# adobe/3D-FM-GAN

Measured on AMD Instinct MI355X. Metric: (photo,render) pairs/sec, higher is better.
Workload: dtype f32; 1 GPU; pairs1024: cfg4 shard: E_Tsr+E_W+E_W_Plus(18 styles) on 256^2 -> co-mod -> Generator(1024) forward, fp32, B=8/GPU; pairs_per_gpu=8, global_pairs=8, image_size=1024, parallelism=replicas x1 (batch-sharded, no collective), launch=eager, ranks=1, full=False

## Files before the change

3d-fm-gan_amd/csrc/modconv_fwd.hip:

```cpp
#include <type_traits>
#include "common.h"
#include <cstdio>
#include <cstdlib>

namespace {

typedef unsigned u32x2 __attribute__((ext_vector_type(2)));

template <int SIZE, typename RSRC>
__device__ __forceinline__ void dma_to_lds(RSRC rsrc, float* lds, unsigned voff, unsigned soff) {
#if defined(__HIP_DEVICE_COMPILE__)
  typedef __attribute__((address_space(3))) void* lds_void_ptr;
  __builtin_amdgcn_raw_ptr_buffer_load_lds(rsrc, (lds_void_ptr)lds, SIZE, voff, soff, 0, 0);
#endif
}

__device__ __forceinline__ const float* uniform_ptr(const float* q) {
  const unsigned long long v = (unsigned long long)q;
  const unsigned lo = __builtin_amdgcn_readfirstlane((unsigned)v), hi = __builtin_amdgcn_readfirstlane((unsigned)(v >> 32));
  return (const float*)(((unsigned long long)hi << 32) | lo);
}
__device__ __forceinline__ unsigned uniform_u32(unsigned v) { return __builtin_amdgcn_readfirstlane(v); }

struct MCParams {
  const float* in; const float* wt; const float* style; const float* demod; float* out;
  int batch, cin, cout, h, w, oh, ow;
  long long out_plane_stride; int out_row_stride;
  struct Seg {
    int m_off, n_off, gh, gw;
    int th, nb, tw_log2;
    int tiles_x, tiles_y, tiles_b;
    unsigned block_end;
    int wide;
  } seg[3];
  int nseg, o_tiles;
  int ksplit, cin_per_split;
  float* ws;
  const float* noise; const float* noise_weight; const float* bias;
  int noise_batch, fuse_act; float alpha, act_scale;
  const float* rgb_wmod;
  const float* rgb_bias; const float* rgb_skip; float* rgb_out;
  int rgb_c;
  int lds_buf_floats, lds_patch_floats;
  int lds_style_floats;
  int debug;
  unsigned long long* dbg_clock;
  int exp_flags;
};

#ifdef FMGAN_EXPERIMENTS
#define MC_DEBUG(p) ((p).debug)
#define MC_CLOCK(p) ((p).dbg_clock)
#define MC_FLAGS(p) ((p).exp_flags)
#else
#define MC_DEBUG(p) 0
#define MC_CLOCK(p) false
#define MC_FLAGS(p) 0
#endif

constexpr int MC_KC = 8;

__device__ __forceinline__ float mc_epilogue(float v, const MCParams& p, float nw, int b, int o, int pix) {
  if (p.demod) v *= p.demod[(long long)b * p.cout + o];
  if (p.fuse_act) {
    const float n = p.noise ? p.noise[(long long)(p.noise_batch == 1 ? 0 : b) * p.oh * p.ow + pix] : 0.f;
    const float bv = p.bias ? p.bias[o] : 0.f;
    v = __fadd_rn(__fadd_rn(v, __fmul_rn(nw, n)), bv);
    v = (v > 0.f ? v : v * p.alpha) * p.act_scale;
  }
  return v;
}

template <int MODE_, int RM_, int RNP_, int WM_, int WN_, int MINB_, int KC_, int PIPE_>
struct TileShape {
  static constexpr int MODE = MODE_, RM = RM_, RNP = RNP_, WM = WM_, WN = WN_, MINB = MINB_, KC = KC_, PIPE = PIPE_;
  static constexpr int BM = 32 * RM * WM, BN = 32 * RNP * WN;
};
struct Plain128x128Reg         : TileShape<   0,  2,   2,  2,  2,    2, MC_KC,    0> {};
struct Plain128x128DmaKc4      : TileShape<   0,  2,   2,  2,  2,    3,     4,    1> {};
struct Plain128x256DmaKc4      : TileShape<   0,  4,   2,  1,  4,    2,     4,    1> {};
struct Plain64x128Reg          : TileShape<   0,  2,   1,  1,  4,    3, MC_KC,    0> {};
struct Plain64x128Dma          : TileShape<   0,  2,   1,  1,  4,    3,     8,    1> {};
struct Plain64x256DmaKc4       : TileShape<   0,  2,   2,  1,  4,    3,     4,    1> {};
struct Plain32x128Reg          : TileShape<   0,  1,   1,  1,  4,    4, MC_KC,    0> {};
struct Plain32x128Dma          : TileShape<   0,  1,   1,  1,  4,    4,     8,    1> {};
struct Plain32x256DmaKc4R128   : TileShape<   0,  1,   2,  1,  4,    4,     4,    1> {};
struct Stride2x128x128Reg      : TileShape<   2,  2,   2,  2,  2,    2, MC_KC,    0> {};
struct Stride2x64x128Reg       : TileShape<   2,  2,   1,  1,  4,    2, MC_KC,    0> {};
struct Stride2x32x128Reg       : TileShape<   2,  1,   1,  1,  4,    2, MC_KC,    0> {};
struct Transposed64x128Reg     : TileShape<   1,  2,   1,  1,  4,    2, MC_KC,    0> {};
struct Transposed64x128Dma     : TileShape<   1,  2,   1,  1,  4,    2,     8,    1> {};
struct Transposed32x128Reg     : TileShape<   1,  1,   1,  1,  4,    3, MC_KC,    0> {};
struct Transposed32x128DmaR128 : TileShape<   1,  1,   1,  1,  4,    4,     8,    1> {};
#ifdef FMGAN_EXPERIMENTS
struct Plain32x256Dma          : TileShape<   0,  1,   2,  1,  4,    3,     8,    1> {};
struct Plain32x256DmaKc4R96    : TileShape<   0,  1,   2,  1,  4,    5,     4,    1> {};
struct Transposed32x256Dma     : TileShape<   1,  1,   2,  1,  4,    2,     8,    1> {};
struct Transposed32x128DmaR170 : TileShape<   1,  1,   1,  1,  4,    3,     8,    1> {};
#endif

template <class Tile, bool RGB>
__global__ __launch_bounds__(256, Tile::MINB) void modconv_mfma_f32(const MCParams p) {
  constexpr int MODE = Tile::MODE, RM = Tile::RM, RNP = Tile::RNP, WM = Tile::WM, WN = Tile::WN, KC = Tile::KC, PIPE = Tile::PIPE;
  static_assert(!RGB || MODE == 0, "the RGB epilogue belongs to the plain conv");
  static_assert(PIPE == 1 || KC == MC_KC, "the register pipeline is built for 8-channel chunks");
  constexpr int BM = Tile::BM;
  constexpr int NPH = MODE == 1 ? 4 : 1;
  static_assert(WM * WN == 4, "4 waves per block");
  extern __shared__ float smem[];
  float* Ws = smem;
  float* Xs = smem + KC * 9 * BM;

  const int tid = threadIdx.x, lane = tid & 63, wave = __builtin_amdgcn_readfirstlane(tid >> 6);
  const int wm = wave / WN, wn = wave % WN;
  const int l31 = lane & 31, khalf = lane >> 5;
  unsigned long long clk0 = 0, rt0 = 0;
  if (MC_CLOCK(p)) { clk0 = __builtin_readcyclecounter(); rt0 = wall_clock64(); }
  if (MC_FLAGS(p) & 1) __builtin_amdgcn_s_setprio(3);

  unsigned lb = xcd_remap(blockIdx.x, gridDim.x);
  int si = 0;
  while (si + 1 < p.nseg && lb >= p.seg[si].block_end) ++si;
  if (si > 0) lb -= p.seg[si - 1].block_end;
  const unsigned tapmask = (MODE == 1 && p.nseg == 3) ? (si == 0 ? 0x1C0u : (si == 1 ? 0x124u : 0x1FFu)) : 0x1FFu;
  const int seg_th = p.seg[si].th, seg_nb = p.seg[si].nb, tw_log2 = p.seg[si].tw_log2;
  const int seg_m_end = p.seg[si].m_off + p.seg[si].gh, seg_n_end = p.seg[si].n_off + p.seg[si].gw;
  constexpr int SP = MODE == 2 ? 2 : 1;
  constexpr int ORG = MODE == 2 ? 0 : 1;
  const bool wide = PIPE == 1 && SP == 1 && p.seg[si].wide != 0;
  const int XORG = wide ? 4 : ORG;
  const int TW = 1 << tw_log2, PWP = wide ? TW + 8 : SP * (TW - 1) + 3;
  const int o_tile = lb % p.o_tiles;
  unsigned pt = lb / p.o_tiles;
  const int tx_i = pt % p.seg[si].tiles_x; pt /= p.seg[si].tiles_x;
  const int ty_i = pt % p.seg[si].tiles_y;
  const int tb_i = pt / p.seg[si].tiles_y;
  const int ks = blockIdx.y;
  const int o0 = o_tile * BM, b0 = tb_i * seg_nb;
  const int x0 = p.seg[si].n_off + tx_i * TW, y0 = p.seg[si].m_off + ty_i * seg_th;
  const int PH = SP * (seg_th - 1) + 3;
  const int plane = PH * PWP;
  const int samp = KC * plane;

  int pbase[RNP], pos_b[RNP], pos_y[RNP], pos_x[RNP];
#pragma unroll
  for (int g = 0; g < RNP; ++g) {
    const int pos = (wn * RNP + g) * 32 + l31;
    const int tx = pos & (TW - 1), r = pos >> tw_log2;
    const int ty = r % seg_th, nbi = r / seg_th;
    pbase[g] = min(nbi, seg_nb - 1) * samp + SP * ty * PWP + SP * tx + (XORG - ORG);
    pos_b[g] = nbi < seg_nb ? b0 + nbi : p.batch; pos_y[g] = y0 + ty; pos_x[g] = x0 + tx;
  }

  f32x16 acc[RM][RNP][NPH];
#pragma unroll
  for (int a = 0; a < RM; ++a)
#pragma unroll
    for (int b = 0; b < RNP; ++b)
#pragma unroll
      for (int c = 0; c < NPH; ++c)
#pragma unroll
        for (int r = 0; r < 16; ++r) acc[a][b][c][r] = 0.f;

  const bool wvec = (p.cout & 3) == 0;
  const int i_begin = ks * p.cin_per_split;
  const int i_end = min(p.cin, i_begin + p.cin_per_split);
  const int hw = p.h * p.w;

  constexpr int BNP = 32 * RNP * WN;
  constexpr int NU = ((SP * (BNP / 32 - 1) + 3) * (SP * 31 + 3) + 255) / 256;
  constexpr int NWV = (KC * 9 * (BM / 4) + 255) / 256;
  const int spatial = seg_nb * plane;
  const float* in_b0 = uniform_ptr(p.in + (long long)b0 * p.cin * hw);
  const float* style_b0 = uniform_ptr(p.style + (long long)b0 * p.cin);
  const bool epi_lds = PIPE == 1 && seg_nb == 1 && p.ksplit == 1;
  float* Es = smem + 2 * p.lds_buf_floats;
  float epi_v = 0.f;
  if constexpr (PIPE == 1) {
    if (epi_lds && tid < 2 * BM) {
      const bool isd = tid >= BM;
      const int oc = min(o0 + (isd ? tid - BM : tid), p.cout - 1);
      epi_v = isd ? 1.f : 0.f;
      if (isd) { if (p.demod) epi_v = p.demod[(long long)min(b0, p.batch - 1) * p.cout + oc]; }
      else if (MODE == 0 && p.fuse_act && p.bias) epi_v = p.bias[oc];
    }
  }
  int gofs[NU], lofs[NU], sofs[NU]; bool inb[NU];
#pragma unroll
  for (int u = 0; u < NU; ++u) {
    const int q = tid + 256 * u;
    const int c = q % PWP;
    int t = q / PWP;
    const int r = t % PH, nbi = t / PH;
    const int b = b0 + nbi, y = SP * y0 + r - ORG, x = SP * x0 + c - ORG;
    inb[u] = q < spatial && b < p.batch && y >= 0 && y < p.h && x >= 0 && x < p.w;
    gofs[u] = inb[u] ? (nbi * p.cin * p.h + y) * p.w + x : 0;
    sofs[u] = nbi * p.cin;
    lofs[u] = q < spatial ? nbi * samp + r * PWP + c : -1;
  }
  float xv[NU][KC];
  f32x4 wv[NWV];
  constexpr long long PARK = 0xFFFFFFF0LL;
  const bool fastw = wvec && o0 + BM <= p.cout && (long long)p.cin * 9 * p.cout * 4 < PARK;
  const bool fastx = (long long)min(seg_nb, p.batch - b0) * p.cin * hw * 4 < PARK;
  const unsigned w_bytes = uniform_u32((unsigned)((long long)p.cin * 9 * p.cout * 4));
  const unsigned x_bytes = uniform_u32((unsigned)((long long)min(seg_nb, p.batch - b0) * p.cin * hw * 4));
  const auto rsrc_w = __builtin_amdgcn_make_buffer_rsrc(const_cast<float*>(p.wt), 0, w_bytes, 0x00020000);
  const auto rsrc_x = __builtin_amdgcn_make_buffer_rsrc(const_cast<float*>(in_b0), 0, x_bytes, 0x00020000);
  unsigned wofs[NWV], xofs[NU];
#pragma unroll
  for (int j = 0; j < NWV; ++j) {
    const int idx = tid + 256 * j;
    const int row = idx / (BM / 4), c4 = idx % (BM / 4);
    wofs[j] = idx < KC * 9 * (BM / 4) ? (unsigned)((row * p.cout + o0 + c4 * 4) * 4) : 0xFFFFFFF0u;
  }
#pragma unroll
  for (int u = 0; u < NU; ++u) xofs[u] = inb[u] ? (unsigned)gofs[u] * 4u : 0xFFFFFFF0u;
  auto issue = [&](int i0) {
    if (fastw && i0 + KC <= i_end) {
      const unsigned soff = (unsigned)(i0 * 9 * p.cout * 4);
#pragma unroll
      for (int j = 0; j < NWV; ++j) {
        const auto t = __builtin_amdgcn_raw_buffer_load_b128(rsrc_w, wofs[j], soff, 0);
        wv[j] = __builtin_bit_cast(f32x4, t);
      }
    } else {
#pragma unroll
      for (int j = 0; j < NWV; ++j) {
        const int idx = tid + 256 * j;
        const int row = idx / (BM / 4), c4 = idx % (BM / 4);
        const int i = i0 + row / 9, o = o0 + c4 * 4;
        f32x4 v = {0.f, 0.f, 0.f, 0.f};
        if (idx < KC * 9 * (BM / 4) && i < i_end) {
          const float* src = p.wt + ((long long)i * 9 + row % 9) * p.cout + o;
          if (wvec && o + 3 < p.cout) {
            v = *reinterpret_cast<const f32x4*>(src);
          } else {
            if (o + 0 < p.cout) v.x = src[0];
            if (o + 1 < p.cout) v.y = src[1];
            if (o + 2 < p.cout) v.z = src[2];
            if (o + 3 < p.cout) v.w = src[3];
          }
        }
        wv[j] = v;
      }
    }
    if (fastx && i0 + KC <= i_end) {
#pragma unroll
      for (int kc = 0; kc < KC; ++kc) {
        const unsigned soff = (unsigned)((i0 + kc) * hw * 4);
#pragma unroll
        for (int u = 0; u < NU; ++u)
          xv[u][kc] = __builtin_bit_cast(float, __builtin_amdgcn_raw_buffer_load_b32(rsrc_x, xofs[u], soff, 0));
      }
    } else {
#pragma unroll
      for (int u = 0; u < NU; ++u)
#pragma unroll
        for (int kc = 0; kc < KC; ++kc) {
          const int i = i0 + kc;
          xv[u][kc] = (inb[u] && i < i_end) ? in_b0[gofs[u] + i * hw] : 0.f;
        }
    }
  };
  auto commit = [&](int i0) {
#pragma unroll
    for (int j = 0; j < NWV; ++j) {
      const int idx = tid + 256 * j;
      if (idx < KC * 9 * (BM / 4)) *reinterpret_cast<f32x4*>(Ws + idx * 4) = wv[j];
    }
#pragma unroll
    for (int u = 0; u < NU; ++u)
      if (lofs[u] >= 0) {
        float sv[KC];
#pragma unroll
        for (int kc = 0; kc < KC; ++kc) sv[kc] = (inb[u] && i0 + kc < i_end) ? style_b0[sofs[u] + i0 + kc] : 0.f;
#pragma unroll
        for (int kc = 0; kc < KC; ++kc) Xs[lofs[u] + kc * plane] = xv[u][kc] * sv[kc];
      }
    for (int q = tid + 256 * NU; q < spatial; q += 256) {
      const int c = q % PWP;
      int t = q / PWP;
      const int r = t % PH, nbi = t / PH;
      const int b = b0 + nbi, y = SP * y0 + r - ORG, x = SP * x0 + c - ORG;
      const bool ok = b < p.batch && y >= 0 && y < p.h && x >= 0 && x < p.w;
      for (int kc = 0; kc < KC; ++kc) {
        const int i = i0 + kc;
        float v = 0.f;
        if (ok && i < i_end) {
          const long long ch = (long long)b * p.cin + i;
          v = p.in[(ch * p.h + y) * p.w + x] * p.style[ch];
        }
        Xs[nbi * samp + kc * plane + r * PWP + c] = v;
      }
    }
  };

  constexpr int NTA = MODE == 1 ? 9 : 3;
  constexpr int NTB = MODE == 1 ? 4 : 3;
  constexpr int NSTAGE = (KC / 2) * (MODE == 1 ? 1 : 3);
  struct Ops { float a[NTA][RM]; float b[NTB][RNP]; float s[RNP]; };
  const float* Wc = Ws;
  const float* Xc = Xs;
  const float* Sc = nullptr;
  int sbase[RNP];
#pragma unroll
  for (int g = 0; g < RNP; ++g) sbase[g] = (pbase[g] / samp) * KC;
  auto fetch = [&](Ops& o, int st) {
    const int kk = MODE == 1 ? st : st / 3, ky = MODE == 1 ? 0 : st % 3;
    const int kc = 2 * kk + khalf;
    const float* wrow = Wc + (kc * 9 + ky * 3) * BM + wm * 32 * RM + l31;
    const float* xrow = Xc + kc * plane;
#pragma unroll
    for (int t = 0; t < NTA; ++t)
#pragma unroll
      for (int m = 0; m < RM; ++m) o.a[t][m] = wrow[t * BM + m * 32];
    if constexpr (PIPE == 1) {
      if (MODE == 1 || ky == 0) {
#pragma unroll
        for (int g = 0; g < RNP; ++g) o.s[g] = Sc[sbase[g] + kc];
      }
    }
#pragma unroll
    for (int j = 0; j < NTB; ++j) {
      const int ro = MODE == 1 ? 1 - (j >> 1) : ky;
      const int co = MODE == 1 ? 1 - (j & 1) : j;
#pragma unroll
      for (int g = 0; g < RNP; ++g) o.b[j][g] = xrow[pbase[g] + ro * PWP + co];
    }
  };
  auto modulate = [&](Ops& o) {
    if constexpr (PIPE == 1) {
#pragma unroll
      for (int j = 0; j < NTB; ++j)
#pragma unroll
        for (int g = 0; g < RNP; ++g) o.b[j][g] *= o.s[g];
    }
  };
  auto mma = [&](const Ops& o, auto all_taps) {
// ... 35 lines not shown
        }
      }
      __builtin_amdgcn_sched_barrier(0);
      modulate(o0);
      __builtin_amdgcn_s_setprio(1);
      mma(o0, all_taps);
      __builtin_amdgcn_s_setprio(0);
      __builtin_amdgcn_sched_barrier(0);
      hook(st + 1);
      if (st + 2 < NSTAGE) {
        fetch(o0, st + 2);
        if constexpr (PIPE == 1 && MODE != 1) {
          if ((st + 2) % 3 != 0) {
#pragma unroll
            for (int g = 0; g < RNP; ++g) o0.s[g] = o1.s[g];
          }
        }
      }
      __builtin_amdgcn_sched_barrier(0);
      modulate(o1);
      __builtin_amdgcn_s_setprio(1);
      mma(o1, all_taps);
      __builtin_amdgcn_s_setprio(0);
      __builtin_amdgcn_sched_barrier(0);
    }
  };

  unsigned long long clk1 = 0, clk2 = 0, clkw = 0, clke = 0, clkl = 0;
  if (MC_CLOCK(p)) clk1 = __builtin_readcyclecounter();
  if (MC_FLAGS(p) & 1) __builtin_amdgcn_s_setprio(0);
  if constexpr (PIPE == 0) {
    if (i_begin < i_end) issue(i_begin);
    for (int i0 = i_begin; i0 < i_end; i0 += KC) {
      const bool live = !(MC_DEBUG(p) & 1) || i0 == i_begin;
      if (!(MC_DEBUG(p) & 2)) __syncthreads();
      if (live) commit(i0);
      if (!(MC_DEBUG(p) & 2)) __syncthreads();
      __builtin_amdgcn_sched_barrier(0);
      if (live && i0 + KC < i_end) issue(i0 + KC);
      contract([](int) {}, std::false_type{});
    }
  } else {
    constexpr unsigned PARKED = 0xFFFFFFF0u;
    constexpr int WSZ = (KC * 9 * BM + 255) / 256 * 256;
    constexpr int WPIECES = WSZ / 256;
    constexpr int NWP = (WPIECES + 3) / 4;
    constexpr int NUP = ((KC * (SP * (BNP / 32 - 1) + 3) * (SP * 31 + 3) + 63) / 64 + 3) / 4;
    const int xs_total = seg_nb * samp;
    const int x_piece_floats = wide ? 256 : 64;
    const int x_pieces = (xs_total + x_piece_floats - 1) / x_piece_floats;
    const int s_pieces = (seg_nb * KC + 63) >> 6;
    const int bstride = p.lds_buf_floats;
    const bool fastc = fastw && fastx;
    const unsigned s_bytes = (unsigned)(min(seg_nb, p.batch - b0) * p.cin * 4);
    const auto rsrc_s = __builtin_amdgcn_make_buffer_rsrc(const_cast<float*>(style_b0), 0, s_bytes, 0x00020000);
    auto x_voff = [&](int e) -> unsigned {
      if (e >= xs_total) return PARKED;
      const int nbi = e / samp, rem = e - nbi * samp;
      const int kc = rem / plane, q = rem - kc * plane;
      const int r = q / PWP, c = q - r * PWP;
      const int b = b0 + nbi, y = SP * y0 + r - ORG, x = SP * x0 + c - XORG;
      const bool ok = b < p.batch && y >= 0 && y < p.h && x >= 0 && x < p.w;
      return ok ? (unsigned)(((nbi * p.cin + kc) * p.h + y) * p.w + x) * 4u : PARKED;
    };
    auto x_voff16 = [&](int g16) -> unsigned { return x_voff(4 * g16); };
    auto s_voff = [&](int e) -> unsigned {
      const int nbi = e / KC, kc = e - nbi * KC;
      return (nbi < seg_nb && b0 + nbi < p.batch) ? (unsigned)(nbi * p.cin + kc) * 4u : PARKED;
    };
    unsigned wvo[NWP], xvo[NUP];
#pragma unroll
    for (int j = 0; j < NWP; ++j) {
      const int idx = (4 * j + wave) * 64 + lane;
      const int row = idx / (BM / 4), c4 = idx % (BM / 4);
      wvo[j] = idx < KC * 9 * (BM / 4) ? (unsigned)((row * p.cout + o0 + c4 * 4) * 4) : PARKED;
    }
#pragma unroll
    for (int u = 0; u < NUP; ++u)
      xvo[u] = 4 * u + wave < x_pieces ? (wide ? x_voff16((4 * u + wave) * 64 + lane) : x_voff((4 * u + wave) * 64 + lane)) : PARKED;
    const unsigned svo = s_voff(wave * 64 + lane);

    constexpr int NPC = NWP + NUP + 1;
    constexpr int PER_STAGE = (NPC + NSTAGE - 1) / NSTAGE;
    auto dma_piece = [&](int k, int i0, int buf) {
      float* Wb = smem + buf * bstride;
      float* Xb = Wb + WSZ;
      const unsigned soff_x = (unsigned)(i0 * hw * 4);
      if (k < NWP) {
        if (4 * k + wave < WPIECES)
          dma_to_lds<16>(rsrc_w, Wb + (4 * k + wave) * 256, wvo[k < NWP ? k : 0], (unsigned)(i0 * 9 * p.cout * 4));
      } else if (k < NWP + NUP) {
        const int u = k - NWP;
        if (4 * u + wave < x_pieces) {
          if (wide) dma_to_lds<16>(rsrc_x, Xb + (4 * u + wave) * 256, xvo[(u >= 0 && u < NUP) ? u : 0], soff_x);
          else dma_to_lds<4>(rsrc_x, Xb + (4 * u + wave) * 64, xvo[(u >= 0 && u < NUP) ? u : 0], soff_x);
        }
      } else {
        float* Sb = Xb + p.lds_patch_floats;
        for (int pc = 4 * NUP + wave; pc < x_pieces; pc += 4) {
          if (wide) dma_to_lds<16>(rsrc_x, Xb + pc * 256, x_voff16(pc * 64 + lane), soff_x);
          else dma_to_lds<4>(rsrc_x, Xb + pc * 64, x_voff(pc * 64 + lane), soff_x);
        }
        if (wave < s_pieces)
          dma_to_lds<4>(rsrc_s, Sb + wave * 64, svo, (unsigned)(i0 * 4));
        for (int pc = 4 + wave; pc < s_pieces; pc += 4)
          dma_to_lds<4>(rsrc_s, Sb + pc * 64, s_voff(pc * 64 + lane), (unsigned)(i0 * 4));
      }
    };
    auto dma_ok = [&](int i0) { return fastc && i0 + KC <= i_end; };

    auto stage = [&](int i0, int buf) {
      float* Wb = smem + buf * bstride;
      float* Xb = Wb + WSZ;
      float* Sb = Xb + p.lds_patch_floats;
      if (dma_ok(i0)) {
#pragma unroll
        for (int k = 0; k < NPC; ++k) dma_piece(k, i0, buf);
      } else {
        for (int idx = tid; idx < KC * 9 * (BM / 4); idx += 256) {
          const int row = idx / (BM / 4), c4 = idx % (BM / 4);
          const int i = i0 + row / 9, o = o0 + c4 * 4;
          f32x4 v = {0.f, 0.f, 0.f, 0.f};
          if (i < i_end) {
            const float* src = p.wt + ((long long)i * 9 + row % 9) * p.cout + o;
            if (o + 0 < p.cout) v.x = src[0];
            if (o + 1 < p.cout) v.y = src[1];
            if (o + 2 < p.cout) v.z = src[2];
            if (o + 3 < p.cout) v.w = src[3];
          }
          *reinterpret_cast<f32x4*>(Wb + idx * 4) = v;
        }
        for (int e = tid; e < x_pieces * x_piece_floats; e += 256) {
          float v = 0.f;
          if (e < xs_total) {
            const int nbi = e / samp, rem = e - nbi * samp;
            const int kc = rem / plane, q = rem - kc * plane;
            const int r = q / PWP, c = q - r * PWP;
            const int b = b0 + nbi, y = SP * y0 + r - ORG, x = SP * x0 + c - XORG, i = i0 + kc;
            if (b < p.batch && y >= 0 && y < p.h && x >= 0 && x < p.w && i < i_end)
              v = p.in[(((long long)b * p.cin + i) * p.h + y) * p.w + x];
          }
          Xb[e] = v;
        }
        for (int e = tid; e < seg_nb * KC; e += 256) {
          const int nbi = e / KC, kc = e - nbi * KC;
          Sb[e] = (b0 + nbi < p.batch && i0 + kc < i_end) ? p.style[(long long)(b0 + nbi) * p.cin + i0 + kc] : 0.f;
        }
      }
    };

    const bool lean = fastc && MC_DEBUG(p) == 0 && i_begin < i_end && ((i_end - i_begin) % KC) == 0 && x_pieces <= 4 * NUP &&
                      s_pieces <= 4 && tapmask == 0x1FFu;
    const bool style_once = lean && seg_nb == 1 && p.lds_style_floats > 0;
    float* Ss = Es + 2 * BM;
    if (lean) {
      auto piece = [&](int k, int i0, int bufi) {
        float* Wb = smem + bufi * bstride;
        float* Xb = Wb + WSZ;
        if (k < NWP) {
          if (WPIECES % 4 == 0 || 4 * k + wave < WPIECES)
            dma_to_lds<16>(rsrc_w, Wb + (4 * k + wave) * 256, wvo[k < NWP ? k : 0], (unsigned)(i0 * 9 * p.cout * 4));
        } else if (k < NWP + NUP) {
          const int u = k - NWP;
          if (4 * u + wave < x_pieces) {
            if (wide) dma_to_lds<16>(rsrc_x, Xb + (4 * u + wave) * 256, xvo[(u >= 0 && u < NUP) ? u : 0], (unsigned)(i0 * hw * 4));
            else dma_to_lds<4>(rsrc_x, Xb + (4 * u + wave) * 64, xvo[(u >= 0 && u < NUP) ? u : 0], (unsigned)(i0 * hw * 4));
          }
        } else if (!style_once && wave < s_pieces) {
          dma_to_lds<4>(rsrc_s, Xb + p.lds_patch_floats + wave * 64, svo, (unsigned)(i0 * 4));
        }
      };
      float sty0 = 0.f, sty1 = 0.f;
      if (style_once) {
        const int n = i_end - i_begin;
        if (tid < n) sty0 = style_b0[i_begin + tid];
        if (tid + 256 < n) sty1 = style_b0[i_begin + tid + 256];
      }
#pragma unroll
      for (int k = 0; k < NPC; ++k) piece(k, i_begin, 0);
      if (epi_lds && tid < 2 * BM) Es[tid] = epi_v;
      if (style_once) {
        if (tid < p.lds_style_floats) Ss[tid] = sty0;
        if (tid + 256 < p.lds_style_floats) Ss[tid + 256] = sty1;
      }
      int bufl = 0;
      for (int i0 = i_begin; i0 < i_end; i0 += KC, bufl ^= 1) {
        const unsigned long long tw0 = MC_CLOCK(p) ? __builtin_readcyclecounter() : 0;
        __builtin_amdgcn_s_waitcnt(0);
        __builtin_amdgcn_s_barrier();
        __builtin_amdgcn_sched_barrier(0);
        if (MC_CLOCK(p)) clkw += __builtin_readcyclecounter() - tw0;
        const int i1 = i0 + KC;
        const bool more = i1 < i_end;
        Wc = smem + bufl * bstride;
        Xc = Wc + WSZ;
        Sc = style_once ? Ss + (i0 - i_begin) : Xc + p.lds_patch_floats;
        contract([&](int st) {
          if (more) {
#pragma unroll
            for (int q = 0; q < PER_STAGE; ++q)
              if (st * PER_STAGE + q < NPC) piece(st * PER_STAGE + q, i1, bufl ^ 1);
          }
        }, std::true_type{});
      }
    }
    if (!lean && i_begin < i_end) {
      stage(i_begin, 0);
      if (epi_lds && tid < 2 * BM) Es[tid] = epi_v;
    }
    int buf = 0;
    for (int i0 = lean ? i_end : i_begin; i0 < i_end; i0 += KC, buf ^= 1) {
      __builtin_amdgcn_s_waitcnt(0);
      if (!(MC_DEBUG(p) & 2)) __builtin_amdgcn_s_barrier();
      __builtin_amdgcn_sched_barrier(0);
      const int i1 = i0 + KC;
      const bool more = i1 < i_end && !(MC_DEBUG(p) & 1);
      const bool spread = more && dma_ok(i1) && !(MC_DEBUG(p) & 4);
      if (more && !spread) stage(i1, buf ^ 1);
      __builtin_amdgcn_sched_barrier(0);
      Wc = smem + buf * bstride;
      Xc = Wc + WSZ;
      Sc = Xc + p.lds_patch_floats;
      contract([&](int st) {
        if (spread) {
#pragma unroll
          for (int q = 0; q < PER_STAGE; ++q)
            if (st * PER_STAGE + q < NPC) dma_piece(st * PER_STAGE + q, i1, buf ^ 1);
        }
      }, std::false_type{});
    }
  }

  if (MC_CLOCK(p)) clk2 = __builtin_readcyclecounter();
  if (MC_FLAGS(p) & 1) __builtin_amdgcn_s_setprio(3);
  const bool partial = p.ksplit > 1;
  const bool actf = MODE == 0 && p.fuse_act && !partial;
  const bool use_demod = p.demod != nullptr && !partial;
  const float nw = (actf && p.noise && p.noise_weight) ? p.noise_weight[0] : 0.f;
  float* dstbase = partial ? p.ws + (long long)ks * p.batch * p.cout * p.oh * p.ow : p.out;
  const long long dps = partial ? (long long)p.oh * p.ow : p.out_plane_stride;
  const int drs = partial ? p.ow : p.out_row_stride;
  const int orow = o0 + wm * 32 * RM + 4 * khalf;
  bool vgs[RNP]; float nzs[RNP];
#pragma unroll
  for (int g = 0; g < RNP; ++g) {
    const int b = pos_b[g], bc = min(b, p.batch - 1);
    if constexpr (MODE != 1) {
      const int y = pos_y[g], x = pos_x[g];
      vgs[g] = b < p.batch && y < p.oh && x < p.ow;
      const int pix = vgs[g] ? y * p.ow + x : 0;
      nzs[g] = (actf && p.noise) ? __fmul_rn(nw, p.noise[(long long)(p.noise_batch == 1 ? 0 : bc) * p.oh * p.ow + pix]) : 0.f;
    } else {
      vgs[g] = b < p.batch && pos_y[g] < seg_m_end && pos_x[g] < seg_n_end;
      nzs[g] = 0.f;
    }
  }
  auto dpos_of = [&](int g) -> float* {
    const int bc = min(pos_b[g], p.batch - 1);
    const int sc = MODE == 1 ? 2 : 1;
    return dstbase + (long long)bc * p.cout * dps + (long long)(vgs[g] ? sc * pos_y[g] : 0) * drs + (vgs[g] ? sc * pos_x[g] : 0);
  };
  const long long slab = (long long)p.cout * dps * 4;
  bool bstore = dstbase != nullptr && o0 + BM <= p.cout && (long long)seg_nb * slab < 0xFFFFFFF0LL;
  if constexpr (MODE == 1) bstore = bstore && 2 * seg_m_end <= p.oh && 2 * seg_n_end <= p.ow;
  unsigned vofs[RNP];
  const float* obase = dstbase ? uniform_ptr(dstbase + (long long)b0 * p.cout * dps) : nullptr;
  const auto rsrc_o = __builtin_amdgcn_make_buffer_rsrc(const_cast<float*>(obase), 0,
      uniform_u32(bstore ? (unsigned)((long long)min(seg_nb, p.batch - b0) * slab) : 0u), 0x00020000);
#pragma unroll
  for (int g = 0; g < RNP; ++g) {
    const long long e = (long long)(pos_b[g] - b0) * p.cout * dps + (long long)(4 * khalf) * dps +
                        (long long)(MODE == 1 ? 2 * pos_y[g] : pos_y[g]) * drs + (MODE == 1 ? 2 * pos_x[g] : pos_x[g]);
    vofs[g] = (bstore && vgs[g]) ? (unsigned)(e * 4) : 0xFFFFFFF0u;
  }
  unsigned alpha_bits = __float_as_uint(p.alpha), ascale_bits = __float_as_uint(p.act_scale);
  asm volatile("" : "+s"(alpha_bits), "+s"(ascale_bits));
  const float alpha = __uint_as_float(alpha_bits), ascale = __uint_as_float(ascale_bits);
  const unsigned dps4 = uniform_u32((unsigned)(dps * 4)), drs4 = uniform_u32((unsigned)drs * 4u);
  if (MC_CLOCK(p)) clke = __builtin_readcyclecounter();
  auto rows = [&](auto act_c, auto bst_c) {
    constexpr bool ACT = decltype(act_c)::value, BST = decltype(bst_c)::value;
#pragma unroll
    for (int m = 0; m < RM; ++m) {
      float bias_m[16], dm_m[16];
      if (epi_lds) {
        const float* eb = Es + (orow - o0) + m * 32;
#pragma unroll
        for (int r = 0; r < 16; ++r) {
          bias_m[r] = ACT ? eb[(r & 3) + 8 * (r >> 2)] : 0.f;
          dm_m[r] = eb[BM + (r & 3) + 8 * (r >> 2)];
        }
      } else {
#pragma unroll
        for (int r = 0; r < 16; ++r) {
          const int oc = min(orow + m * 32 + (r & 3) + 8 * (r >> 2), p.cout - 1);
          bias_m[r] = (ACT && p.bias) ? p.bias[oc] : 0.f;
          dm_m[r] = 1.f;
        }
      }
      const unsigned so_m = (unsigned)(o0 + wm * 32 * RM + m * 32) * dps4;
#pragma unroll
      for (int g = 0; g < RNP; ++g) {
        const int bc = min(pos_b[g], p.batch - 1);
        if (!epi_lds && use_demod && (g == 0 || seg_nb > 1)) {
#pragma unroll
          for (int r = 0; r < 16; ++r)
            dm_m[r] = p.demod[(long long)bc * p.cout + min(orow + m * 32 + (r & 3) + 8 * (r >> 2), p.cout - 1)];
        }
        const bool vg = vgs[g];
        float* dpos = BST ? nullptr : dpos_of(g);
        if (MC_CLOCK(p) && m == 0 && g == 0) {
          __builtin_amdgcn_sched_barrier(0);
          __builtin_amdgcn_s_waitcnt(0);
          clkl = __builtin_readcyclecounter();
          __builtin_amdgcn_sched_barrier(0);
        }
        if constexpr (MODE != 1) {
          const float nz = nzs[g];
#pragma unroll
          for (int r = 0; r < 16; ++r) {
            const int o = orow + m * 32 + (r & 3) + 8 * (r >> 2);
            float v = acc[m][g][0][r] * dm_m[r];
            if constexpr (ACT) {
              v = __fadd_rn(__fadd_rn(v, nz), bias_m[r]);
              v = (v > 0.f ? v : v * alpha) * ascale;
            }
            if constexpr (BST) {
              if constexpr (RGB) acc[m][g][0][r] = vg ? v : 0.f;
              __builtin_amdgcn_raw_buffer_store_b32(__float_as_uint(v), rsrc_o, vofs[g], so_m + (unsigned)((r & 3) + 8 * (r >> 2)) * dps4, 0);
            } else {
              if constexpr (RGB) acc[m][g][0][r] = (vg && o < p.cout) ? v : 0.f;
              if ((!RGB || dstbase) && vg && o < p.cout) dpos[(long long)o * dps] = v;
            }
          }
        } else {
          const int X = 2 * pos_x[g], Y0 = 2 * pos_y[g];
          const bool pair = X + 1 < p.ow;
#pragma unroll
          for (int r = 0; r < 16; ++r) {
            const int o = orow + m * 32 + (r & 3) + 8 * (r >> 2);
            if constexpr (BST) {
#pragma unroll
              for (int py = 0; py < 2; ++py) {
                u32x2 t;
                t.x = __float_as_uint(acc[m][g][py * 2][r] * dm_m[r]);
                t.y = __float_as_uint(acc[m][g][py * 2 + 1][r] * dm_m[r]);
                __builtin_amdgcn_raw_buffer_store_b64(t, rsrc_o, vofs[g], so_m + (unsigned)((r & 3) + 8 * (r >> 2)) * dps4 + (unsigned)py * drs4, 0);
              }
            } else {
              if (!(vg && o < p.cout)) continue;
              float* dst = dpos + (long long)o * dps;
#pragma unroll
              for (int py = 0; py < 2; ++py) {
                if (Y0 + py >= p.oh) continue;
                const float v0 = acc[m][g][py * 2][r] * dm_m[r], v1 = acc[m][g][py * 2 + 1][r] * dm_m[r];
                if (pair) {
                  f32x2_u t; t.x = v0; t.y = v1;
                  *reinterpret_cast<f32x2_u*>(dst + (long long)py * drs) = t;
                } else {
                  dst[(long long)py * drs] = v0;
                }
              }
            }
          }
        }
      }
    }
  };
  if (bstore) {
    if (actf) rows(std::true_type{}, std::true_type{}); else rows(std::false_type{}, std::true_type{});
  } else {
    if (actf) rows(std::true_type{}, std::false_type{}); else rows(std::false_type{}, std::false_type{});
  }
  if (MC_CLOCK(p) && tid == 0 && (blockIdx.x & 63) == 0) {
    const unsigned long long clk3 = __builtin_readcyclecounter();
    atomicAdd(p.dbg_clock, clk3 - clk0);
    atomicAdd(p.dbg_clock + 1, wall_clock64() - rt0);
    atomicAdd(p.dbg_clock + 2, clk1 - clk0);
    atomicAdd(p.dbg_clock + 3, clk2 - clk1);
    atomicAdd(p.dbg_clock + 4, clk3 - clk2);
    atomicAdd(p.dbg_clock + 5, 1ULL);
    atomicAdd(p.dbg_clock + 8, clkl - clke);
    __builtin_amdgcn_s_waitcnt(0);
    atomicAdd(p.dbg_clock + 9, __builtin_readcyclecounter() - clk3);
    atomicAdd(p.dbg_clock + 7, clke - clk2);
    atomicAdd(p.dbg_clock + 6, clkw);
  }
  if constexpr (RGB) {
    float rs[RNP][3];
#pragma unroll
    for (int g = 0; g < RNP; ++g) rs[g][0] = rs[g][1] = rs[g][2] = 0.f;
    const float* wmod = p.rgb_wmod + (long long)min(b0, p.batch - 1) * 3 * p.cout;
#pragma unroll
    for (int m = 0; m < RM; ++m) {
      float rw[3][16];
#pragma unroll
      for (int r = 0; r < 16; ++r) {
        const int oc = min(orow + m * 32 + (r & 3) + 8 * (r >> 2), p.cout - 1);
#pragma unroll
        for (int c = 0; c < 3; ++c) rw[c][r] = wmod[c * p.cout + oc];
      }
#pragma unroll
      for (int g = 0; g < RNP; ++g)
#pragma unroll
        for (int r = 0; r < 16; ++r)
#pragma unroll
          for (int c = 0; c < 3; ++c) rs[g][c] = fmaf(acc[m][g][0][r], rw[c][r], rs[g][c]);
    }
#pragma unroll
    for (int g = 0; g < RNP; ++g)
#pragma unroll
      for (int c = 0; c < 3; ++c) rs[g][c] += __shfl_xor(rs[g][c], 32, 64);
    if constexpr (WM > 1) {
      static_assert(WM == 2, "two output-channel waves at most");
      __syncthreads();
      float* red = smem + ((wn * RNP) * 3) * 32;
      if (wm == 1 && khalf == 0)
#pragma unroll
        for (int g = 0; g < RNP; ++g)
#pragma unroll
          for (int c = 0; c < 3; ++c) red[(g * 3 + c) * 32 + l31] = rs[g][c];
      __syncthreads();
      if (wm == 0 && khalf == 0)
#pragma unroll
        for (int g = 0; g < RNP; ++g)
#pragma unroll
          for (int c = 0; c < 3; ++c) rs[g][c] += red[(g * 3 + c) * 32 + l31];
    }
    if (wm == 0 && khalf == 0) {
#pragma unroll
      for (int g = 0; g < RNP; ++g) {
        const int b = pos_b[g], y = pos_y[g], x = pos_x[g];
        if (b >= p.batch || y >= p.oh || x >= p.ow) continue;
#pragma unroll
        for (int c = 0; c < 3; ++c) {
          if (c >= p.rgb_c) continue;
          const long long off = (((long long)b * p.rgb_c + c) * p.oh + y) * p.ow + x;
          float v = rs[g][c];
          if (p.rgb_bias) v = __fadd_rn(v, p.rgb_bias[c]);
          if (p.rgb_skip) v = __fadd_rn(v, p.rgb_skip[off]);
          p.rgb_out[off] = v;
        }
      }
    }
  }
}

__global__ __launch_bounds__(256) void modconv_splitk_finish_f32(const MCParams p) {
  const float nw = (p.fuse_act && p.noise && p.noise_weight) ? p.noise_weight[0] : 0.f;
  const int hw = p.oh * p.ow;
  const long long total = (long long)p.batch * p.cout * hw;
  for (long long idx = (long long)blockIdx.x * blockDim.x + threadIdx.x; idx < total;
       idx += (long long)gridDim.x * blockDim.x) {
    float v = 0.f;
    for (int ks = 0; ks < p.ksplit; ++ks) v += p.ws[ks * total + idx];
    const int pix = (int)(idx % hw);
    const long long bo = idx / hw;
    p.out[bo * p.out_plane_stride + (long long)(pix / p.ow) * p.out_row_stride + pix % p.ow] =
        mc_epilogue(v, p, nw, (int)(bo / p.cout), (int)(bo % p.cout), pix);
  }
}

inline int pick_tw_log2(int gw, int gh) {
  if (gh <= 32 && gw <= 2) return gw <= 1 ? 0 : 1;
  return gw <= 4 ? 2 : (gw <= 8 ? 3 : (gw <= 16 ? 4 : 5));
}

inline bool mc_wide_patch() {
#ifdef FMGAN_EXPERIMENTS
  const char* e = getenv("FMGAN_MC_WIDE");
  return !(e && e[0] == '0');
#else
  return true;
#endif
}

inline long long plan_segment(MCParams::Seg& sg, int batch, int BN) {
  sg.tw_log2 = pick_tw_log2(sg.gw, sg.gh);
  const int TW = 1 << sg.tw_log2;
  const int rows_total = BN / TW;
  int th = rows_total, nb = 1;
  if (sg.gh < rows_total) {
    th = 1;
    while (th < sg.gh) th <<= 1;
    nb = rows_total / th;
  }
  sg.th = th; sg.nb = nb;
  sg.tiles_x = (sg.gw + TW - 1) / TW;
  sg.tiles_y = (sg.gh + th - 1) / th;
  sg.tiles_b = (batch + nb - 1) / nb;
  return (long long)sg.tiles_x * sg.tiles_y * sg.tiles_b;
}

constexpr size_t MC_LDS_LIMIT = 64 * 1024;
constexpr size_t MC_LDS_MAX = 160 * 1024;

struct MCPick {
  int cfg; char variant; int bm, bn, ksplit;
};

template <class Tile, bool FUSES_RGB>
int launch_tile(MCParams& p, hipStream_t s, bool plan_only) {
  constexpr int MODE = Tile::MODE, MINB = Tile::MINB, KC = Tile::KC, PIPE = Tile::PIPE, BM = Tile::BM, BN = Tile::BN;
  static_assert(!FUSES_RGB || MODE == 0, "the RGB epilogue belongs to the plain conv");
  if constexpr (!FUSES_RGB) { if (p.rgb_out) return FMGAN_EUNSUPPORTED; }
  constexpr int SP = MODE == 2 ? 2 : 1;
  p.o_tiles = (p.cout + BM - 1) / BM;
  long long blocks = 0;
  size_t patch = 0, nbmax = 1;
  auto patch_floats = [&](const MCParams::Seg& sg) {
    size_t f = (size_t)sg.nb * KC * (SP * (sg.th - 1) + 3) * (sg.wide ? (1 << sg.tw_log2) + 8 : SP * ((1 << sg.tw_log2) - 1) + 3);
    return sg.wide ? (f + 255) / 256 * 256 : f;
  };
  long long seg_blocks[3] = {0, 0, 0};
  int main_seg = 0;
  for (int i = 0; i < p.nseg; ++i) {
    seg_blocks[i] = plan_segment(p.seg[i], p.batch, BN);
    if (seg_blocks[i] > seg_blocks[main_seg]) main_seg = i;
    p.seg[i].wide = PIPE == 1 && SP == 1 && p.seg[i].tw_log2 == 5 && (p.seg[i].n_off & 3) == 0 && (p.w & 3) == 0 &&
                    (reinterpret_cast<uintptr_t>(p.in) & 15) == 0 && mc_wide_patch();
  }
  const size_t main_patch = patch_floats(p.seg[main_seg]);
  const bool cap_strips = seg_blocks[main_seg] * p.o_tiles >= 4LL * FMGAN_NUM_CU;
  for (int i = 0; i < p.nseg; ++i) {
    MCParams::Seg& sg = p.seg[i];
    while (cap_strips && i != main_seg && patch_floats(sg) > main_patch && (sg.nb > 1 || sg.th > 1)) {
      if (sg.nb > 1) sg.nb >>= 1; else sg.th >>= 1;
      sg.tiles_y = (sg.gh + sg.th - 1) / sg.th;
      sg.tiles_b = (p.batch + sg.nb - 1) / sg.nb;
      seg_blocks[i] = (long long)sg.tiles_x * sg.tiles_y * sg.tiles_b;
    }
    blocks += seg_blocks[i] * p.o_tiles;
    if (blocks > 0x7fffffffLL) return FMGAN_EOVERFLOW;
    sg.block_end = (unsigned)blocks;
    const int nb_live = sg.nb < p.batch ? sg.nb : p.batch;
    if ((long long)nb_live * p.cin * p.h * p.w >= (1LL << 31)) return FMGAN_EOVERFLOW;
    const size_t f = patch_floats(sg);
    if (f > patch) patch = f;
    if ((size_t)sg.nb > nbmax) nbmax = sg.nb;
  }
  size_t lds = sizeof(float) * ((size_t)KC * 9 * BM + patch);
  if constexpr (PIPE == 1) {
    if (p.cin_per_split % KC != 0) return 1;
    p.lds_patch_floats = (int)((patch + 63) / 64 * 64);
    p.lds_buf_floats = (KC * 9 * BM + 255) / 256 * 256 + p.lds_patch_floats + (int)((nbmax * KC + 63) / 64 * 64);
    p.lds_style_floats = (nbmax == 1 && p.cin_per_split <= 512) ? p.cin_per_split : 0;
    lds = sizeof(float) * (2 * (size_t)p.lds_buf_floats + 2 * BM + p.lds_style_floats);
    if (lds > (MINB == 1 ? MC_LDS_MAX : MC_LDS_LIMIT)) return 1;
    if (lds > MC_LDS_LIMIT && !plan_only) {
      static bool raised = false;
      if (!raised) {
        if (hipFuncSetAttribute(reinterpret_cast<const void*>(&modconv_mfma_f32<Tile, false>),
                                hipFuncAttributeMaxDynamicSharedMemorySize, (int)MC_LDS_MAX) != hipSuccess) {
          (void)hipGetLastError();
          return 1;
        }
        raised = true;
      }
    }
  }
  if constexpr (FUSES_RGB) {
    if (p.rgb_out) {
      if (p.o_tiles != 1 || p.ksplit != 1) return FMGAN_EUNSUPPORTED;
      if (nbmax > 1) return PIPE == 1 ? 1 : FMGAN_EUNSUPPORTED;
      if (plan_only) return FMGAN_OK;
      hipLaunchKernelGGL((modconv_mfma_f32<Tile, true>), dim3((unsigned)blocks, 1), dim3(256), lds, s, p);
      return fmgan_check_launch();
    }
  }
  if (plan_only) return FMGAN_OK;
  hipLaunchKernelGGL((modconv_mfma_f32<Tile, false>), dim3((unsigned)blocks, p.ksplit), dim3(256), lds, s, p);
  return fmgan_check_launch();
}

struct TileEntry {
  int mode, cfg;
  char variant;
  int BM, BN;
  bool fuses_rgb;
  int (*launch)(MCParams&, hipStream_t, bool plan_only);
};
template <class Tile, bool FUSES_RGB = false>
constexpr TileEntry tile_entry(int cfg, char variant) {
  return {Tile::MODE, cfg, variant, Tile::BM, Tile::BN, FUSES_RGB, &launch_tile<Tile, FUSES_RGB>};
}
#ifdef FMGAN_EXPERIMENTS
constexpr bool MC_EXP = true;
#else
constexpr bool MC_EXP = false;
#endif
constexpr TileEntry MC_TILES[] = {
    tile_entry<Plain128x256DmaKc4>(0, 'C'),
    tile_entry<Plain128x128DmaKc4, MC_EXP>(0, 'B'),
    tile_entry<Plain128x128Reg, true>(0, 'A'),
    tile_entry<Plain64x256DmaKc4>(1, 'C'),
    tile_entry<Plain64x128Dma, MC_EXP>(1, 'B'),
    tile_entry<Plain64x128Reg, true>(1, 'A'),
    tile_entry<Plain32x256DmaKc4R128, true>(2, 'E'),
    tile_entry<Plain32x128Dma, true>(2, 'B'),
    tile_entry<Plain32x128Reg, true>(2, 'A'),
#ifdef FMGAN_EXPERIMENTS
    tile_entry<Plain32x256Dma, true>(2, 'C'),
    tile_entry<Plain32x256DmaKc4R96, true>(2, 'D'),
#endif
    tile_entry<Transposed64x128Dma>(1, 'B'),
    tile_entry<Transposed64x128Reg>(1, 'A'),
    tile_entry<Transposed32x128DmaR128>(2, 'D'),
    tile_entry<Transposed32x128Reg>(2, 'A'),
#ifdef FMGAN_EXPERIMENTS
    tile_entry<Transposed32x256Dma>(1, 'C'),
    tile_entry<Transposed32x128DmaR170>(2, 'B'),
    tile_entry<Transposed32x256Dma>(2, 'C'),
#endif
    tile_entry<Stride2x128x128Reg>(0, 'A'),
    tile_entry<Stride2x64x128Reg>(1, 'A'),
    tile_entry<Stride2x32x128Reg>(2, 'A'),
};

inline const TileEntry* find_tile(int mode, int cfg, char variant) {
  for (const TileEntry& e : MC_TILES)
    if (e.mode == mode && e.cfg == cfg && e.variant == variant) return &e;
  return nullptr;
}

inline char mc_variant(int mode, int cfg) {
  char v = 'A';
  for (const TileEntry& e : MC_TILES)
    if (e.mode == mode && e.cfg == cfg) { v = e.variant; break; }
#ifdef FMGAN_EXPERIMENTS
  char name[32];
  snprintf(name, sizeof(name), "FMGAN_MC_V%d%d", mode, cfg);
  const char* e = getenv(name);
  if (e && e[0] >= 'A' && e[0] <= 'E') v = e[0];
#endif
  return v;
}

inline int pick_cfg(int mode, int cout, long long positions) {
  if (mode == 0) {
    if (positions <= 2048) return 2;
    return cout >= 96 ? 0 : (cout >= 48 ? 1 : 2);
  }
  if (mode == 2) return cout >= 96 ? 0 : (cout >= 48 ? 1 : 2);
  if (cout >= 192 && positions >= 4096) return 2;
  return cout >= 48 ? 1 : 2;
}

inline void model_tile_dims(int mode, int cfg, int& BM, int& BN) {
  (void)mode;
  const int bm[3] = {128, 64, 32};
  BM = bm[cfg]; BN = 128;
}

inline int model_blocks_per_cu(int mode, int cfg) {
  if (mode == 1) return cfg == 2 ? 3 : 2;
  return cfg == 0 ? 2 : (cfg == 1 ? (mode == 0 ? 3 : 2) : 4);
}

inline long long blocks_with(const MCParams& p, int BM, int BN) {
  long long blocks = 0;
  for (int i = 0; i < p.nseg; ++i) {
    MCParams::Seg sg = p.seg[i];
    blocks += plan_segment(sg, p.batch, BN);
  }
  return blocks * ((p.cout + BM - 1) / BM);
}

inline int launch_any(int mode, int cfg, MCParams& p, hipStream_t s, MCPick* pick = nullptr) {
  char v = mc_variant(mode, cfg);
  const TileEntry* e = nullptr;
  if (mode == 0 && v == 'C' && (e = find_tile(0, cfg, 'C')) != nullptr) {
    const bool small = p.ksplit > 1 || blocks_with(p, e->BM, e->BN) < 2LL * FMGAN_NUM_CU;
    if (cfg < 2 && (small || p.rgb_out)) v = (!p.rgb_out && (long long)p.batch * p.h * p.w >= 1536) ? 'B' : 'A';
    else if (cfg == 2 && small) v = 'B';
  }
  if (mode == 0 && (v == 'D' || v == 'E') && (e = find_tile(0, 2, v)) != nullptr) {
    const bool small = p.ksplit > 1 || blocks_with(p, e->BM, e->BN) < 2LL * FMGAN_NUM_CU;
    if (small) v = 'B';
  }
  int st = 1;
  if (v != 'A' && (e = find_tile(mode, cfg, v)) != nullptr) st = e->launch(p, s, pick != nullptr);
  if (st == 1) {
    e = find_tile(mode, cfg, 'A');
    st = e ? e->launch(p, s, pick != nullptr) : FMGAN_EUNSUPPORTED;
  }
  if (pick && st == FMGAN_OK) *pick = {cfg, e->variant, e->BM, e->BN, p.ksplit};
  return st;
}

inline void out_dims(int mode, int h, int w, int& oh, int& ow) {
  if (mode == 1) { oh = 2 * h + 1; ow = 2 * w + 1; }
  else if (mode == 2) { oh = (h - 3) / 2 + 1; ow = (w - 3) / 2 + 1; }
  else { oh = h; ow = w; }
}

inline long long count_blocks(int mode, int cfg, int batch, int cout, int h, int w) {
  int BM, BN;
  model_tile_dims(mode, cfg, BM, BN);
  if (mode == 2) out_dims(2, h, w, h, w);
  MCParams::Seg sg[3] = {{0, 0, h, w}, {h, 0, 1, w + 1}, {0, w, h, 1}};
// ... 192 lines not shown
```

Baseline: 398.8 pairs/s.

## Stage toRGB weights in LDS and skip dead stores in fused RGB epilogue

The fused modconv+toRGB epilogue now preloads the per-channel RGB modulation weights into LDS alongside bias/demod and reads them as vector loads, replacing scattered global loads per accumulator row. When the feature map output is not needed (rgb-only), the per-element buffer stores are compiled out. Tile position decoding uses shifts instead of division and is recomputed late to cut register pressure, and rgb_skip/bias are prefetched before the reduction. It costs more LDS per block, which could lower occupancy or push some tile configs past the LDS limit.

```diff
diff --git a/3d-fm-gan_amd/csrc/modconv_fwd.hip b/3d-fm-gan_amd/csrc/modconv_fwd.hip
--- a/3d-fm-gan_amd/csrc/modconv_fwd.hip
+++ b/3d-fm-gan_amd/csrc/modconv_fwd.hip
@@ -142,14 +142,18 @@
   const int plane = PH * PWP;
   const int samp = KC * plane;
 
-  int pbase[RNP], pos_b[RNP], pos_y[RNP], pos_x[RNP];
+  const int th_log2 = __builtin_ctz((unsigned)seg_th);
+  auto tile_pos = [&](int g, int l, int& tx, int& ty, int& nbi) {
+    const int pos = (wn * RNP + g) * 32 + l;
+    const int r = pos >> tw_log2;
+    tx = pos & (TW - 1); ty = r & (seg_th - 1); nbi = r >> th_log2;
+  };
+  int pbase[RNP];
 #pragma unroll
   for (int g = 0; g < RNP; ++g) {
-    const int pos = (wn * RNP + g) * 32 + l31;
-    const int tx = pos & (TW - 1), r = pos >> tw_log2;
-    const int ty = r % seg_th, nbi = r / seg_th;
+    int tx, ty, nbi;
+    tile_pos(g, l31, tx, ty, nbi);
     pbase[g] = min(nbi, seg_nb - 1) * samp + SP * ty * PWP + SP * tx + (XORG - ORG);
-    pos_b[g] = nbi < seg_nb ? b0 + nbi : p.batch; pos_y[g] = y0 + ty; pos_x[g] = x0 + tx;
   }
 
   f32x16 acc[RM][RNP][NPH];
@@ -173,18 +177,31 @@
   const int spatial = seg_nb * plane;
   const float* in_b0 = uniform_ptr(p.in + (long long)b0 * p.cin * hw);
   const float* style_b0 = uniform_ptr(p.style + (long long)b0 * p.cin);
-  const bool epi_lds = PIPE == 1 && seg_nb == 1 && p.ksplit == 1;
+  const bool epi_lds = PIPE == 1 && (RGB || (seg_nb == 1 && p.ksplit == 1));
   float* Es = smem + 2 * p.lds_buf_floats;
-  float epi_v = 0.f;
+  constexpr int EPI_N = (RGB ? 5 : 2) * BM;
+  constexpr int NEV = (EPI_N + 255) / 256;
+  float epi_v[NEV];
+#pragma unroll
+  for (int j = 0; j < NEV; ++j) epi_v[j] = 0.f;
   if constexpr (PIPE == 1) {
-    if (epi_lds && tid < 2 * BM) {
-      const bool isd = tid >= BM;
-      const int oc = min(o0 + (isd ? tid - BM : tid), p.cout - 1);
-      epi_v = isd ? 1.f : 0.f;
-      if (isd) { if (p.demod) epi_v = p.demod[(long long)min(b0, p.batch - 1) * p.cout + oc]; }
-      else if (MODE == 0 && p.fuse_act && p.bias) epi_v = p.bias[oc];
-    }
-  }
+#pragma unroll
+    for (int j = 0; j < NEV; ++j) {
+      const int idx = tid + 256 * j;
+      if (epi_lds && idx < EPI_N) {
+        const int sec = idx / BM, oraw = o0 + idx % BM, oc = min(oraw, p.cout - 1);
+        const long long bc = min(b0, p.batch - 1);
+        if (sec == 0) { if (MODE == 0 && p.fuse_act && p.bias) epi_v[j] = p.bias[oc]; }
+        else if (sec == 1) epi_v[j] = p.demod ? p.demod[bc * p.cout + oc] : 1.f;
+        else if constexpr (RGB) { if (oraw < p.cout) epi_v[j] = p.rgb_wmod[(bc * 3 + (sec - 2)) * p.cout + oc]; }
+      }
+    }
+  }
+  auto epi_commit = [&]() {
+#pragma unroll
+    for (int j = 0; j < NEV; ++j)
+      if (epi_lds && tid + 256 * j < EPI_N) Es[tid + 256 * j] = epi_v[j];
+  };
   int gofs[NU], lofs[NU], sofs[NU]; bool inb[NU];
 #pragma unroll
   for (int u = 0; u < NU; ++u) {
@@ -526,7 +543,7 @@
     const bool lean = fastc && MC_DEBUG(p) == 0 && i_begin < i_end && ((i_end - i_begin) % KC) == 0 && x_pieces <= 4 * NUP &&
                       s_pieces <= 4 && tapmask == 0x1FFu;
     const bool style_once = lean && seg_nb == 1 && p.lds_style_floats > 0;
-    float* Ss = Es + 2 * BM;
+    float* Ss = Es + EPI_N;
     if (lean) {
       auto piece = [&](int k, int i0, int bufi) {
         float* Wb = smem + bufi * bstride;
@@ -552,7 +569,7 @@
       }
 #pragma unroll
       for (int k = 0; k < NPC; ++k) piece(k, i_begin, 0);
-      if (epi_lds && tid < 2 * BM) Es[tid] = epi_v;
+      epi_commit();
       if (style_once) {
         if (tid < p.lds_style_floats) Ss[tid] = sty0;
         if (tid + 256 < p.lds_style_floats) Ss[tid + 256] = sty1;
@@ -580,7 +597,7 @@
     }
     if (!lean && i_begin < i_end) {
       stage(i_begin, 0);
-      if (epi_lds && tid < 2 * BM) Es[tid] = epi_v;
+      epi_commit();
     }
     int buf = 0;
     for (int i0 = lean ? i_end : i_begin; i0 < i_end; i0 += KC, buf ^= 1) {
@@ -607,6 +624,17 @@
 
   if (MC_CLOCK(p)) clk2 = __builtin_readcyclecounter();
   if (MC_FLAGS(p) & 1) __builtin_amdgcn_s_setprio(3);
+  int pos_b[RNP], pos_y[RNP], pos_x[RNP];
+  {
+    int l31e = l31;
+    if constexpr (MODE == 1) asm volatile("" : "+v"(l31e));
+#pragma unroll
+    for (int g = 0; g < RNP; ++g) {
+      int tx, ty, nbi;
+      tile_pos(g, l31e, tx, ty, nbi);
+      pos_b[g] = nbi < seg_nb ? b0 + nbi : p.batch; pos_y[g] = y0 + ty; pos_x[g] = x0 + tx;
+    }
+  }
   const bool partial = p.ksplit > 1;
   const bool actf = MODE == 0 && p.fuse_act && !partial;
   const bool use_demod = p.demod != nullptr && !partial;
@@ -652,8 +680,8 @@
   const float alpha = __uint_as_float(alpha_bits), ascale = __uint_as_float(ascale_bits);
   const unsigned dps4 = uniform_u32((unsigned)(dps * 4)), drs4 = uniform_u32((unsigned)drs * 4u);
   if (MC_CLOCK(p)) clke = __builtin_readcyclecounter();
-  auto rows = [&](auto act_c, auto bst_c) {
-    constexpr bool ACT = decltype(act_c)::value, BST = decltype(bst_c)::value;
+  auto rows = [&](auto act_c, auto bst_c, auto sto_c) {
+    constexpr bool ACT = decltype(act_c)::value, BST = decltype(bst_c)::value, STO = decltype(sto_c)::value;
 #pragma unroll
     for (int m = 0; m < RM; ++m) {
       float bias_m[16], dm_m[16];
@@ -682,7 +710,7 @@
             dm_m[r] = p.demod[(long long)bc * p.cout + min(orow + m * 32 + (r & 3) + 8 * (r >> 2), p.cout - 1)];
         }
         const bool vg = vgs[g];
-        float* dpos = BST ? nullptr : dpos_of(g);
+        float* drow = BST ? nullptr : dpos_of(g) + (long long)(orow + m * 32) * dps;
         if (MC_CLOCK(p) && m == 0 && g == 0) {
           __builtin_amdgcn_sched_barrier(0);
           __builtin_amdgcn_s_waitcnt(0);
@@ -701,10 +729,11 @@
             }
             if constexpr (BST) {
               if constexpr (RGB) acc[m][g][0][r] = vg ? v : 0.f;
-              __builtin_amdgcn_raw_buffer_store_b32(__float_as_uint(v), rsrc_o, vofs[g], so_m + (unsigned)((r & 3) + 8 * (r >> 2)) * dps4, 0);
+              if constexpr (STO)
+                __builtin_amdgcn_raw_buffer_store_b32(__float_as_uint(v), rsrc_o, vofs[g], so_m + (unsigned)((r & 3) + 8 * (r >> 2)) * dps4, 0);
             } else {
               if constexpr (RGB) acc[m][g][0][r] = (vg && o < p.cout) ? v : 0.f;
-              if ((!RGB || dstbase) && vg && o < p.cout) dpos[(long long)o * dps] = v;
+              if ((!RGB || dstbase) && vg && o < p.cout) drow[(long long)((r & 3) + 8 * (r >> 2)) * dps] = v;
             }
           }
         } else {
@@ -723,7 +752,7 @@
               }
             } else {
               if (!(vg && o < p.cout)) continue;
-              float* dst = dpos + (long long)o * dps;
+              float* dst = drow + (long long)((r & 3) + 8 * (r >> 2)) * dps;
 #pragma unroll
               for (int py = 0; py < 2; ++py) {
                 if (Y0 + py >= p.oh) continue;
@@ -741,10 +770,15 @@
       }
     }
   };
+  const bool rgb_only = RGB && dstbase == nullptr && o0 + BM <= p.cout;
+  constexpr std::true_type yes{};
+  constexpr std::false_type no{};
   if (bstore) {
-    if (actf) rows(std::true_type{}, std::true_type{}); else rows(std::false_type{}, std::true_type{});
+    if (actf) rows(yes, yes, yes); else rows(no, yes, yes);
+  } else if (rgb_only) {
+    if constexpr (RGB) { if (actf) rows(yes, yes, no); else rows(no, yes, no); }
   } else {
-    if (actf) rows(std::true_type{}, std::false_type{}); else rows(std::false_type{}, std::false_type{});
+    if (actf) rows(yes, no, yes); else rows(no, no, yes);
   }
   if (MC_CLOCK(p) && tid == 0 && (blockIdx.x & 63) == 0) {
     const unsigned long long clk3 = __builtin_readcyclecounter();
@@ -764,23 +798,44 @@
     float rs[RNP][3];
 #pragma unroll
     for (int g = 0; g < RNP; ++g) rs[g][0] = rs[g][1] = rs[g][2] = 0.f;
-    const float* wmod = p.rgb_wmod + (long long)min(b0, p.batch - 1) * 3 * p.cout;
-#pragma unroll
-    for (int m = 0; m < RM; ++m) {
-      float rw[3][16];
-#pragma unroll
-      for (int r = 0; r < 16; ++r) {
-        const int oc = min(orow + m * 32 + (r & 3) + 8 * (r >> 2), p.cout - 1);
-#pragma unroll
-        for (int c = 0; c < 3; ++c) rw[c][r] = wmod[c * p.cout + oc];
-      }
-#pragma unroll
-      for (int g = 0; g < RNP; ++g)
-#pragma unroll
-        for (int r = 0; r < 16; ++r)
-#pragma unroll
-          for (int c = 0; c < 3; ++c) rs[g][c] = fmaf(acc[m][g][0][r], rw[c][r], rs[g][c]);
-    }
+    const float* Rs = Es + 2 * BM;
+    if constexpr (PIPE == 0) {
+      __syncthreads();
+      const float* wmod = p.rgb_wmod + (long long)min(b0, p.batch - 1) * 3 * p.cout;
+      for (int idx = tid; idx < 3 * BM; idx += 256) {
+        const int oraw = o0 + idx % BM;
+        smem[idx] = oraw < p.cout ? wmod[(idx / BM) * p.cout + oraw] : 0.f;
+      }
+      __syncthreads();
+      Rs = smem;
+    }
+    const long long rplane = (long long)p.oh * p.ow;
+    long long roff[RNP];
+    float rsk[RNP][3];
+#pragma unroll
+    for (int g = 0; g < RNP; ++g) {
+      roff[g] = vgs[g] ? (((long long)pos_b[g] * p.rgb_c) * p.oh + pos_y[g]) * p.ow + pos_x[g] : 0;
+#pragma unroll
+      for (int c = 0; c < 3; ++c) rsk[g][c] = (p.rgb_skip && c < p.rgb_c) ? p.rgb_skip[roff[g] + c * rplane] : 0.f;
+    }
+    float rbias[3];
+#pragma unroll
+    for (int c = 0; c < 3; ++c) rbias[c] = (p.rgb_bias && c < p.rgb_c) ? p.rgb_bias[c] : 0.f;
+    const float* rrow = Rs + wm * 32 * RM + 4 * khalf;
+#pragma unroll
+    for (int m = 0; m < RM; ++m)
+#pragma unroll
+      for (int q = 0; q < 4; ++q) {
+        f32x4 w4[3];
+#pragma unroll
+        for (int c = 0; c < 3; ++c) w4[c] = *reinterpret_cast<const f32x4*>(rrow + c * BM + m * 32 + 8 * q);
+#pragma unroll
+        for (int g = 0; g < RNP; ++g)
+#pragma unroll
+          for (int j = 0; j < 4; ++j)
+#pragma unroll
+            for (int c = 0; c < 3; ++c) rs[g][c] = fmaf(acc[m][g][0][4 * q + j], w4[c][j], rs[g][c]);
+      }
 #pragma unroll
     for (int g = 0; g < RNP; ++g)
 #pragma unroll
@@ -804,16 +859,14 @@
     if (wm == 0 && khalf == 0) {
 #pragma unroll
       for (int g = 0; g < RNP; ++g) {
-        const int b = pos_b[g], y = pos_y[g], x = pos_x[g];
-        if (b >= p.batch || y >= p.oh || x >= p.ow) continue;
+        if (!vgs[g]) continue;
 #pragma unroll
         for (int c = 0; c < 3; ++c) {
           if (c >= p.rgb_c) continue;
-          const long long off = (((long long)b * p.rgb_c + c) * p.oh + y) * p.ow + x;
           float v = rs[g][c];
-          if (p.rgb_bias) v = __fadd_rn(v, p.rgb_bias[c]);
-          if (p.rgb_skip) v = __fadd_rn(v, p.rgb_skip[off]);
-          p.rgb_out[off] = v;
+          if (p.rgb_bias) v = __fadd_rn(v, rbias[c]);
+          if (p.rgb_skip) v = __fadd_rn(v, rsk[g][c]);
+          p.rgb_out[roff[g] + c * rplane] = v;
         }
       }
     }
@@ -919,7 +972,7 @@
     p.lds_patch_floats = (int)((patch + 63) / 64 * 64);
     p.lds_buf_floats = (KC * 9 * BM + 255) / 256 * 256 + p.lds_patch_floats + (int)((nbmax * KC + 63) / 64 * 64);
     p.lds_style_floats = (nbmax == 1 && p.cin_per_split <= 512) ? p.cin_per_split : 0;
-    lds = sizeof(float) * (2 * (size_t)p.lds_buf_floats + 2 * BM + p.lds_style_floats);
+    lds = sizeof(float) * (2 * (size_t)p.lds_buf_floats + (p.rgb_out ? 5 : 2) * BM + p.lds_style_floats);
     if (lds > (MINB == 1 ? MC_LDS_MAX : MC_LDS_LIMIT)) return 1;
     if (lds > MC_LDS_LIMIT && !plan_only) {
       static bool raised = false;
```

After: 397.0 pairs/s. No clear change (-0.4%).
